# genometools/vstree

Hardware: AMD Instinct MI355X
Metric: queries/sec (100 bp queries, vmatch -mum -l 20 semantics, 3 Gbp ESA index resident in HBM) (higher is better)
Workload: dtype u8; 1 GPU; 3 Gbp synthetic DNA index, 10 M x 100 bp queries per GPU, -mum -l 20; index_bp=3000000000, queries_per_gpu=10000000, query_len=100, minlen=20, prefixlength=13, index_bytes_hbm=115012207262, reads_in_hbm=two bits per symbol, 32 bytes per read (vsa_pack_reads), parallelism=index replicated, queries sharded x1

## Files before the change

vstree_amd/csrc/api.hip:

```cpp
#include "vsa_internal.hpp"
#include <atomic>
#include <thread>
#include <time.h>
#include <algorithm>

static thread_local char g_errbuf[VSA_ERRBUF_SIZE] = "";

extern "C" char *vsa_errbuf()
{
  return g_errbuf;
}

extern "C" const char *vsa_messagespace(void)
{
  return g_errbuf;
}

int vsa_set_device(int device)
{
  VSA_HIP(hipSetDevice(device));
  return 0;
}

extern "C" int vsa_device_count(void)
// ... 411 lines not shown
    const void *from;
    uint64_t bytes;
    bool allocate;
  };
  const uint64_t ncodes = src->D > 0 ? 1ull << (2 * src->D) : 0,
                 nblocks = (n >> 6) + 1, nwaves = (nblocks + 63) / 64;
  Piece pieces[] = {
      {(void **) &ix->tis_alloc, src->tis_alloc,
       VSA_TIS_FRONTPAD + n + VSA_TIS_BACKPAD, false},
      {&ix->suf, src->suf, (n + 1) * src->isize, false},
      {(void **) &ix->lcp, src->lcp, n + 1 + 32, false},
      {&ix->llv, src->llv, 2 * src->nllv * src->isize, false},
      {&ix->bck, src->bck, 2 * src->numofcodes * src->isize, false},
      {(void **) &ix->bwt, src->bwt, n + 1 + 32, false},
      {(void **) &ix->esa8, src->esa8, (n + 1) * 8 + 64, true},
      {(void **) &ix->bck2, src->bck2, 2 * ncodes * 4 + 16, true},
      {(void **) &ix->slot16, src->slot16,
       (uint64_t) src->slotwords * ncodes * 8 + 32, true},
      {(void **) &ix->tis2, src->tis2, nblocks * 16 + 64, true},
      {(void **) &ix->spec64, src->spec64, nwaves * 8 + 64, true}};
  for (const Piece &p : pieces)
  {
    if (p.from == nullptr || p.bytes == 0)
    {
      continue;
    }
    if (p.allocate)
    {
      if (vsa_hip_malloc(p.dst, p.bytes) != hipSuccess)
      {
        VSA_ERROR("vsa_index_clone: out of device memory");
        return fail(-100);
      }
      ix->device_bytes += p.bytes;
    }
    const hipError_t e =
        hipMemcpyPeerAsync(*p.dst, device, p.from, src->device, p.bytes,
                           ix->stream);
    if (e != hipSuccess)
    {
      VSA_ERROR("vsa_index_clone: copy from device %d to device %d: %s",
                src->device, device, hipGetErrorString(e));
      return fail(-100);
    }
  }
  if (hipStreamSynchronize(ix->stream) != hipSuccess)
  {
    VSA_ERROR("vsa_index_clone: copy failed");
    return fail(-100);
  }
  ix->device_bytes = src->device_bytes;
  ix->D = src->D;
  ix->tune = src->tune;
  ix->qspeedup = src->qspeedup;
  ix->slotwords = src->slotwords;
  ix->firstspecial = src->firstspecial;
  ix->querysepposition = src->querysepposition;
  ix->hasindexedqueries = src->hasindexedqueries;
  ix->lcpquirk = src->lcpquirk;
  *clone = ix;
  return 0;
}

extern "C" void vsa_index_close(vsa_index *ix)
{
  if (ix == nullptr)
  {
    return;
  }
  (void) hipSetDevice(ix->device);
  (void) hipFree(ix->tis_alloc);
  (void) hipFree(ix->suf);
  (void) hipFree(ix->lcp);
  (void) hipFree(ix->llv);
  (void) hipFree(ix->bck);
  (void) hipFree(ix->bwt);
  (void) hipFree(ix->esa8);
  (void) hipFree(ix->bck2);
  (void) hipFree(ix->slot16);
  (void) hipFree(ix->tis2);
  (void) hipFree(ix->spec64);
  (void) hipFree(ix->isa32);
  (void) hipFree(ix->repbits);
  if (ix->stream != nullptr)
  {
    vsa_dev_forget_stream(ix->stream);
    (void) hipStreamDestroy(ix->stream);
  }
  delete ix;
}

extern "C" int vsa_index_from_tables(const vsa_tables *t, int device,
                                     vsa_index **index)
{
  if (t == nullptr || index == nullptr)
  {
    VSA_ERROR("vsa_index_from_tables: NULL argument");
    return -1;
  }
  *index = nullptr;
  if (t->integersize != 32 && t->integersize != 64)
  {
    VSA_ERROR("integersize=%u: only 32 and 64 bit indexes are supported",
              t->integersize);
    return -2;
  }
// ... 1009 lines not shown
```

vstree_amd/csrc/esa_search.hip:

```cpp
#include "search_host.hpp"
#include <rocprim/rocprim.hpp>
#include <type_traits>

#include "search_complete.inc"
#include "search_query.inc"
#include "mum_workplan.inc"
#include "mem_workplan.inc"
#include "mum_filter.inc"
#include "candidate_sort.inc"
#include <atomic>


namespace
{


enum class Form
{
  Ref,
  Deep,
  Staged,
  Rows,
  Windows
};
// ... 425 lines not shown
  rf->recsize = rf->valbits != 0 ? 4 : (rf->packed ? 8 : sizeof(vsa_match));
  return 0;
}

int compact_into(const RecordForm &form, DevBuf &raw, DevBuf &rawkeys,
                 uint64_t cap, DevBuf &cursors, DevBuf &doff, DevBuf &out,
                 DevBuf &keys, uint64_t at, hipStream_t stream)
{
  auto launch = [&](auto rec) {
    using REC = decltype(rec);
    k_compact_shards<REC><<<VSA_CURSOR_SHARDS, VSA_BLOCK, 0, stream>>>(
        raw.as<REC>(), rawkeys.as<uint64_t>(), cap,
        cursors.as<unsigned long long>(), doff.as<uint64_t>(),
        out.as<REC>() + at, keys.as<uint64_t>() + at);
  };
  if (form.valbits != 0)
  {
    launch(uint32_t());
  } else if (form.packed)
  {
    launch(uint64_t());
  } else
  {
    launch(vsa_match());
  }
  VSA_HIP(hipGetLastError());
  return 0;
}

struct QueryRun
{
  const vsa_index *index;
  const vsa_queries *queries;
  hipStream_t stream;
  DevQueries qs;
  bool domum, domumcand, ordered;
  uint32_t searchlength;
  RecordForm rec;
  Timer tall, tsearch, tfirst;
  DevBuf base;
  const uint64_t *dbase = nullptr;
  uint32_t perquery = 0;
  uint64_t nitems = 0;
  bool reduce = false, memplan = false;
  Form form = Form::Ref;
  DevBuf wcount, wtemp, wplan, wlist, wfirste, wfmlen, wfmdb, wboffset;
  const uint64_t *nlistword = nullptr;
  DevBuf pcursor, pdoff, psummary, prawout, prawkeys;
  uint64_t pcap = 0;
  bool fromplan = false, planemit = false;
  uint64_t plansearches = 0;
  DevBuf cursor, doff, summary, blocksum, rtemp, rawout, rawkeys, out, keys;
  uint64_t shardcap = 0, needed = 0, nplan = 0, nfirst = 0, plannedwork = 0;
  double searchms = 0;

  QueryRun(const vsa_index *ix, const vsa_queries *q, bool mum, bool cand,
           bool ord, uint32_t least)
      : index(ix), queries(q), stream(ix->stream), qs(devqueries(q)),
        domum(mum), domumcand(cand), ordered(ord), searchlength(least),
        tall(stream), tsearch(stream), tfirst(stream)
  {
  }
};

template <typename IDX>
int workitems(QueryRun &st)
{
  const uint64_t nqr = st.queries->nq, least = st.searchlength;
  if (st.qs.uniformlen != 0)
  {
    st.perquery = (st.qs.uniformlen >= least) ? st.qs.uniformlen - least + 1
                                              : 0;
    st.nitems = (uint64_t) st.perquery * nqr;
    return 0;
  }
  DevBuf btemp;
  auto items = rocprim::make_transform_iterator(
      rocprim::counting_iterator<uint64_t>(0),
      [len = st.qs.length, nqr, least] __device__(uint64_t q) -> uint64_t {
        if (q >= nqr)
        {
          return 0;
        }
        const uint64_t l = len[q];
        return l >= least ? l - least + 1 : 0;
      });
  if (st.base.alloc((nqr + 1) * 8))
  {
    return -100;
  }
  VSA_HIP(rocprim_run(btemp, [&](void *p, size_t &tb) {
    return rocprim::exclusive_scan(p, tb, items, st.base.as<uint64_t>(),
                                   (uint64_t) 0, (size_t) (nqr + 1),
                                   rocprim::plus<uint64_t>(), st.stream);
  }));
  st.dbase = st.base.as<uint64_t>();
  const Fetch f = {st.dbase + nqr, 8};
  return fetchwords(st.stream, &f, 1, &st.nitems) ? -100 : 0;
}

int decide(QueryRun &st)
{
  const vsa_index *index = st.index;
  const vsa_queries *queries = st.queries;
  const uint64_t maxoffsets =
      (queries->maxlength >= st.searchlength)
// ... 171 lines not shown
  if (first_pass(st, ix, st.form, bcount.as<uint64_t>()))
  {
    return -100;
  }
  VSA_HIP(rocprim_run(st.wtemp, [&](void *p, size_t &tb) {
    return rocprim::exclusive_scan(p, tb, bcount.as<uint64_t>(),
                                   st.wboffset.as<uint64_t>(), (uint64_t) 0,
                                   (size_t) (nb + 1), rocprim::plus<uint64_t>(),
                                   st.stream);
  }));
  k_wanted_fill<<<vsa_grid(nb), VSA_BLOCK, 0, st.stream>>>(
      st.wcount.as<uint32_t>(), nq, 0u, st.wboffset.as<uint64_t>(),
      st.wlist.as<uint32_t>());
  VSA_HIP(hipGetLastError());
  st.nlistword = st.wboffset.as<uint64_t>() + nb;
  PlanEmit em = PlanEmit();
  if (st.form != Form::Ref && plan_emit(st, VSA_PLAN_ROUNDS - 1, &em))
  {
    return -100;
  }
  withform(st.form, [&](auto deep, auto, auto rows, auto) {
    k_mum_plan<IDX, deep, deep, rows><<<gridfor(nq), VSA_BLOCK, 0, st.stream>>>(
        ix, st.qs, st.wlist.as<uint32_t>(), st.nlistword, st.searchlength,
        st.wfirste.as<uint32_t>(), st.wcount.as<uint32_t>(),
        st.wplan.as<PlanRanges>(), em);
  });
  if (st.planemit)
  {
    VSA_HIP(plan_summary(st));
  }
  VSA_HIP(hipGetLastError());
  const char *pf = getenv("VSA_DEBUG_PLANFILE");
  if (pf != nullptr && dump_planfile(st, pf))
  {
    return -100;
  }
  st.fromplan = true;
  return 0;
}

template <typename IDX>
void launch_search(QueryRun &st, const DevIndex<IDX> &ix,
                   uint64_t nplanblocks)
{
  withform(st.form, [&](auto deep, auto, auto rows, auto) {
    auto planned = [&](auto mum) {
      k_query_search_planned<IDX, 256, deep, rows, mum>
          <<<vsa_grid(nplanblocks), 256, 0, st.stream>>>(
              ix, st.qs, st.dbase, st.perquery, st.wplan.as<PlanRanges>(),
              st.wcount.as<uint32_t>(), st.searchlength,
              st.rawout.as<vsa_match>(), st.rawkeys.as<uint64_t>(),
              st.shardcap, VSA_CURSOR_SHARDS - 1,
              st.cursor.as<unsigned long long>(), st.rec.packbits,
              st.rec.valbits, st.blocksum.as<unsigned long long>());
    };
    auto unplanned = [&](auto mum) {
      k_query_search<IDX, mum, deep, 256>
          <<<vsa_grid((st.nitems + 255) / 256), 256, 0, st.stream>>>(
              ix, st.qs, st.dbase, st.perquery, st.nitems, st.searchlength,
              st.rawout.as<vsa_match>(), st.rawkeys.as<uint64_t>(),
              st.shardcap, VSA_CURSOR_SHARDS - 1,
              st.cursor.as<unsigned long long>(), st.rec.packbits,
              st.rec.valbits);
    };
    if (st.fromplan && st.domum)
    {
      planned(std::true_type());
    } else if (st.fromplan)
    {
      if constexpr (deep && !rows)
      {
        planned(std::false_type());
      }
    } else if (st.nitems > 0 && st.domum)
    {
      unplanned(std::true_type());
    } else if (st.nitems > 0)
    {
      unplanned(std::false_type());
    }
  });
}

template <typename IDX>
int search(QueryRun &st, const DevIndex<IDX> &ix)
{
  const uint32_t nshards = VSA_CURSOR_SHARDS;
  const uint64_t nplanblocks = (st.queries->nq + 255) / 256;
  size_t rbytes = 0;
  if (st.fromplan)
  {
    if (st.blocksum.alloc((vsa_grid_blocks(nplanblocks) + 1) * 8))
    {
      return -100;
    }
    VSA_HIP(rocprim::reduce(nullptr, rbytes,
                            st.blocksum.as<unsigned long long>(),
                            (unsigned long long *) nullptr, 0ull,
                            (size_t) nplanblocks,
                            rocprim::plus<unsigned long long>(), st.stream));
    if (st.rtemp.alloc(rbytes))
    {
      return -100;
    }
  }
  if (st.cursor.alloc((size_t) nshards * VSA_CURSOR_STRIDE * 8) ||
      st.doff.alloc(nshards * 8) || st.summary.alloc(5 * 8))
  {
    return -100;
  }
  st.shardcap =
      std::max<uint64_t>((st.queries->nq * 2 / nshards) * 5 / 4 + 64, 256);
  uint64_t maxshard = 0;
  for (int attempt = 0; attempt < 2; attempt++)
  {
    if (st.rawout.alloc(nshards * st.shardcap * st.rec.recsize) ||
        st.rawkeys.alloc(nshards * st.shardcap * 8))
    {
      return -100;
    }
    VSA_HIP(hipMemsetAsync(st.cursor.p, 0,
                           (size_t) nshards * VSA_CURSOR_STRIDE * 8,
                           st.stream));
    st.tsearch.start();
    launch_search(st, ix, nplanblocks);
    st.tsearch.stop();
    VSA_HIP(hipGetLastError());
    if (st.fromplan)
    {
      VSA_HIP(rocprim::reduce(st.rtemp.p, rbytes,
                              st.blocksum.as<unsigned long long>(),
                              st.summary.as<unsigned long long>() + 4, 0ull,
                              (size_t) nplanblocks,
                              rocprim::plus<unsigned long long>(), st.stream));
    }
    const uint64_t *sm = st.summary.as<uint64_t>();
    VSA_HIP(shard_summary(st.cursor.as<unsigned long long>(), nshards,
                          st.doff.as<uint64_t>(), st.summary.as<uint64_t>(),
                          st.stream));
    const Fetch f[7] = {{sm, 8}, {sm + 1, 8}, {sm + 2, 8}, {sm + 3, 8},
                        {sm + 4, 8}, {st.planemit ? st.psummary.p : sm, 8},
                        {st.nlistword != nullptr ? st.nlistword : sm, 8}};
    uint64_t got[7];
    if (fetchwords(st.stream, f, 7, got))
    {
      return -100;
    }
    if (st.nlistword != nullptr)
    {
      st.nfirst = got[6] >> 32;
      st.plansearches = 2 * (got[6] & 0xFFFFFFFFull);
    }
    st.nplan = st.planemit ? got[5] : 0;
    st.needed = got[0];
    maxshard = got[1];
    st.plannedwork = st.fromplan ? got[4] : 0;
    st.searchms += st.tsearch.ms();
    if (maxshard <= st.shardcap)
    {
      return 0;
    }
    st.shardcap = maxshard;
  }
  VSA_ERROR("match buffer overflow: %llu > %llu",
            (unsigned long long) maxshard, (unsigned long long) st.shardcap);
  return -5;
}

int compact(QueryRun &st)
{
  const uint64_t total = st.needed + st.nplan + st.nfirst;
  if (total == 0)
  {
    return 0;
  }
  if (st.out.alloc(total * st.rec.recsize) || st.keys.alloc(total * 8) ||
      (st.nplan > 0 &&
       compact_into(st.rec, st.prawout, st.prawkeys, st.pcap, st.pcursor,
                    st.pdoff, st.out, st.keys, st.needed, st.stream)) ||
      (st.needed > 0 &&
       compact_into(st.rec, st.rawout, st.rawkeys, st.shardcap, st.cursor,
                    st.doff, st.out, st.keys, 0, st.stream)))
  {
    return -100;
  }
  if (st.nfirst > 0)
  {
    k_append_first<<<gridfor(st.queries->nq), VSA_BLOCK, 0, st.stream>>>(
        st.wfmlen.as<uint32_t>(), st.wfmdb.as<uint64_t>(),
        st.wboffset.as<uint64_t>(), st.queries->nq, st.perquery, st.dbase,
        st.qs.seqoffset, st.needed + st.nplan, st.out.as<vsa_match>(),
        st.keys.as<uint64_t>(), st.rec.packbits, st.rec.valbits);
    VSA_HIP(hipGetLastError());
  }
  st.needed = total;
  return 0;
}

#define VSA_CS_MINPAIRS (1u << 14)

std::atomic<uint64_t> g_cs_runs{0}, g_cs_overflows{0}, g_cs_longruns{0},
    g_cs_shift{0}, g_cs_buckets{0};

bool feedsbuckets(const QueryRun &st)
{
  const uint64_t total = st.needed + st.nplan + st.nfirst;
  const uint32_t tune = st.index->tune;
  if (!(st.domum && !st.domumcand && st.rec.packed && (tune & 4u) == 0 &&
        total > 0 && (total >= VSA_CS_MINPAIRS || (tune & 8u) != 0) &&
// ... 146 lines not shown
                  bitsfor(st.nitems), st.stream))
    {
      return -100;
    }
    res->count = needed;
    res->matches = (vsa_match *) sm.release();
  }
  return 0;
}

template <typename IDX>
int run_query(const vsa_index *index, const vsa_queries *queries, bool domum,
              bool domumcand, uint32_t searchlength, vsa_result *res,
              bool ordered = true, uint32_t forcebits = 0)
{
  vsa_dev_set_stream(index->stream);
  QueryRun st(index, queries, domum, domumcand, ordered, searchlength);
  const DevIndex<IDX> ix = index->view<IDX>();
  if (workitems<IDX>(st))
  {
    return -100;
  }
  res->stats.searches = st.nitems;
  if (st.nitems == 0)
  {
    return 0;
  }
  st.tall.start();
  if (const int rc = recordform(index, queries, domum, domumcand, ordered,
                                forcebits, &st.rec))
  {
    return rc;
  }
  if (decide(st) || (st.memplan && mem_plan(st, ix)) ||
      (st.reduce && mum_plan(st, ix)))
  {
    return -100;
  }
  if (const int rc = search(st, ix))
  {
    return rc;
  }
  uint64_t mumsum = ~0ull;
  if (finish(st, res, &mumsum))
  {
    return -100;
  }
  st.tall.stop();
  VSA_HIP(hipStreamSynchronize(st.stream));
  res->stats.count = res->count;
  res->stats.search_kernel_ms = st.searchms;
  res->stats.anchor_ms = 0;
  res->stats.first_kernel_ms = st.tfirst.ms();
  res->stats.kernel_searches = st.fromplan ? st.plannedwork : st.nitems;
  if (st.fromplan)
  {
    res->stats.searches = st.plannedwork + queries->nq + st.plansearches;
  }
  res->stats.total_device_ms = st.tall.ms();
  if (mumsum != ~0ull)
  {
    res->stats.sumlength = mumsum;
    return 0;
  }
  if (st.rec.keeppairs)
  {
    res->stats.sumlength = 0;
    return 0;
  }
  return sumlengths(res->matches, res->count, st.stream,
                    &res->stats.sumlength);
}

template <typename Limits, typename Run>
int query_entry(const char *name, const vsa_index *index,
                const vsa_queries *queries, const uint64_t *searchlength,
                vsa_result **result, Limits limits, Run run)
{
  if (index == nullptr || queries == nullptr || result == nullptr)
  {
    VSA_ERROR("%s: NULL argument", name);
    return -1;
  }
  *result = nullptr;
  if (queries->device != index->device)
  {
    VSA_ERROR("queries live on device %d, index on device %d",
              queries->device, index->device);
    return -1;
  }
  if (index->bck == nullptr)
  {
    VSA_ERROR("table bck is not loaded");
    return -3;
  }
  if (searchlength != nullptr && *searchlength < index->pl)
  {
    VSA_ERROR("searchlength=%lu must be >= %lu=prefixlen",
              (unsigned long) *searchlength, (unsigned long) index->pl);
    return -2;
  }
  if (const int rc = limits())
  {
    return rc;
  }
  if (vsa_set_device(index->device) != 0)
  {
// ... 331 lines not shown
```

vstree_amd/csrc/index_derive.hip:

```cpp
#include "search_host.hpp"
#include <rocprim/rocprim.hpp>


template <typename IDX>
__global__ void __launch_bounds__(VSA_BLOCK)
k_make_esa8(const uint8_t *__restrict__ tis, const IDX *__restrict__ suf,
            const uint8_t *__restrict__ lcp, uint64_t count, uint32_t D,
            uint64_t *__restrict__ esa8)
{
  const uint64_t j = vsa_bid() * VSA_BLOCK + threadIdx.x;
  if (j >= count)
  {
    return;
  }
  const uint64_t s = suf[j];
  const uint8_t *t = tis + s + D;
  uint64_t key = 0, flag = 0;
#pragma unroll
  for (uint32_t k = 0; k < VSA_KEYSYMS; k++)
  {
    const uint8_t a = t[k];
    if (VSA_ISSPECIAL(a))
    {
      flag = VSA_KEYFLAG;
// ... 33 lines not shown
      const uint64_t packed = vsa_pack16(v.lo, v.hi);
      out[k >> 1] |= packed << (32 * (1 - (k & 1)));
    }
    out[0] = __builtin_bswap64(out[0]);
    out[1] = __builtin_bswap64(out[1]);
    reinterpret_cast<uint64_t *>(tis2)[2 * b] = out[0];
    reinterpret_cast<uint64_t *>(tis2)[2 * b + 1] = out[1];
    special = firstbad != ~0ull || 64 * b + 64 > n;
    if (firstbad != ~0ull)
    {
      atomicMin(firstspecial, (unsigned long long) firstbad);
    }
  }
  const uint64_t mask = __ballot(special);
  if ((threadIdx.x & 63) == 0 && b < nblocks)
  {
    reinterpret_cast<uint64_t *>(spec64)[b >> 6] = mask;
  }
}

template <int W, typename IDX>
__global__ void __launch_bounds__(VSA_BLOCK)
k_make_slots(const IDX *__restrict__ bck2, const uint64_t *__restrict__ esa8,
             uint64_t ncodes, uint64_t *__restrict__ slot,
             unsigned int *__restrict__ toobig)
{
  for (uint64_t c = vsa_bid() * VSA_BLOCK + threadIdx.x;
       c < ncodes; c += vsa_nblocks() * VSA_BLOCK)
  {
    const IDX left = bck2[2 * c], mid = bck2[2 * c + 1];
    if constexpr (sizeof(IDX) == 4)
    {
      slot[W * c] = (uint64_t) left | ((uint64_t) mid << 32);
    } else
    {
      const uint64_t cnt = mid > left ? mid - left : 0;
      if (cnt >> (64 - VSA_WIDE_LEFTBITS) != 0)
      {
        *toobig = 1;
      }
      slot[W * c] = left | (cnt << VSA_WIDE_LEFTBITS);
    }
#pragma unroll
    for (int k = 0; k + 1 < W; k++)
    {
      slot[W * c + 1 + k] = (mid > left + k) ? esa8[left + k] : 0;
    }
  }
}

int vsa_index_make_esa8(vsa_index *ix)
{
  const char *off = getenv("VSA_NO_ESA8");
  if (ix->esa8 != nullptr)
  {
    (void) hipFree(ix->esa8);
    ix->esa8 = nullptr;
  }
  if (ix->bck2 != nullptr)
  {
    (void) hipFree(ix->bck2);
    ix->bck2 = nullptr;
  }
  if (ix->slot16 != nullptr)
  {
    (void) hipFree(ix->slot16);
    ix->slot16 = nullptr;
  }
  if (ix->tis2 != nullptr)
  {
    (void) hipFree(ix->tis2);
    (void) hipFree(ix->spec64);
    ix->tis2 = ix->spec64 = nullptr;
  }
  const bool wide = ix->isize != 4;
  if (ix->numofchars != 4 || ix->bck == nullptr ||
      (wide && ((ix->n + 1) >> VSA_WIDE_LEFTBITS) != 0) ||
      (off != nullptr && strcmp(off, "1") == 0))
  {
    return 0;
  }
  uint32_t D = 1;
  while (D < 16 && (1ull << (2 * D)) < ix->n)
  {
    D++;
  }
  if (D < ix->pl)
  {
    D = ix->pl;
  }
  const char *fd = getenv("VSA_DEEP_PREFIX");
  if (fd != nullptr && atoi(fd) >= (int) ix->pl && atoi(fd) <= 16)
  {
    D = (uint32_t) atoi(fd);
  } else
  {
    size_t freeb = 0, totalb = 0;
    const uint32_t wanted = D;
    (void) hipStreamSynchronize(ix->stream);
    vsa_dev_trim();
    while (D > ix->pl && D > 12 &&
           hipMemGetInfo(&freeb, &totalb) == hipSuccess)
    {
      const uint64_t codes = 1ull << (2 * D),
                     need = 16 * codes + 2 * codes * ix->isize +
                            8 * (ix->n + 1) + ix->n / 4 + totalb / 10;
      if (need <= freeb)
      {
        break;
      }
      D--;
    }
    const char *tr = getenv("VSA_TRACE");
    if (tr != nullptr && strcmp(tr, "0") != 0)
    {
      fprintf(stderr, "vstree_amd: derived tables: deep prefix %u (wanted %u; "
              "%.1f GB free of %.1f on the device)\n", D, wanted,
              (double) freeb / 1e9, (double) totalb / 1e9);
    }
  }
  if (D > 16)
  {
    return 0;
  }
  static_assert(VSA_TIS_BACKPAD >= 16 + VSA_KEYSYMS + 8, "text pad too small");
  ix->D = D;
  const char *tune = getenv("VSA_TUNE");
  ix->tune = tune != nullptr ? (uint32_t) atoi(tune) : 0;
  const uint64_t count = ix->n + 1, ncodes = 1ull << (2 * D);
  VSA_HIP(hipStreamSynchronize(ix->stream));
  vsa_dev_trim();
  if (vsa_hip_malloc((void **) &ix->slot16, 2 * ncodes * 8 + 32) != hipSuccess)
  {
    (void) hipGetLastError();
    ix->slot16 = nullptr;
    ix->D = 0;
    return 0;
  }
  VSA_HIP(vsa_hip_malloc((void **) &ix->bck2, 2 * ncodes * ix->isize + 16));
  VSA_HIP(vsa_hip_malloc((void **) &ix->esa8, count * 8 + 64));
  ix->device_bytes += count * 8 + 2 * ncodes * ix->isize;
  if (wide ? vsa_build_bucket_table(ix->tis_alloc + VSA_TIS_FRONTPAD, ix->n,
                                    (const uint64_t *) ix->suf, D, 4,
                                    (uint64_t *) ix->bck2, ix->stream)
           : vsa_build_bucket_table(ix->tis_alloc + VSA_TIS_FRONTPAD, ix->n,
                                    (const uint32_t *) ix->suf, D, 4,
                                    ix->bck2, ix->stream))
  {
    return -100;
  }
  if (wide)
  {
    k_make_esa8<uint64_t><<<gridfor(count), VSA_BLOCK, 0, ix->stream>>>(
        ix->tis_alloc + VSA_TIS_FRONTPAD, (const uint64_t *) ix->suf, ix->lcp,
        count, D, ix->esa8);
  } else
  {
    k_make_esa8<uint32_t><<<gridfor(count), VSA_BLOCK, 0, ix->stream>>>(
        ix->tis_alloc + VSA_TIS_FRONTPAD, (const uint32_t *) ix->suf, ix->lcp,
        count, D, ix->esa8);
  }
  VSA_HIP(hipGetLastError());
  VSA_HIP(hipStreamSynchronize(ix->stream));
  {
    static_assert(VSA_TIS_BACKPAD >= 64, "text pad too small for k_pack_text");
    const uint64_t nblocks = (ix->n >> 6) + 1,
                   nwaves = (nblocks + 63) / 64;
    unsigned long long *dfirst = nullptr, hfirst = ix->n;
    VSA_HIP(vsa_hip_malloc((void **) &ix->tis2, nblocks * 16 + 64));
    VSA_HIP(vsa_hip_malloc((void **) &ix->spec64, nwaves * 8 + 64));
    VSA_HIP(vsa_hip_malloc((void **) &dfirst, 8));
    VSA_HIP(hipMemsetAsync(ix->tis2 + nblocks * 16, 0, 64, ix->stream));
    VSA_HIP(hipMemsetAsync(ix->spec64 + nwaves * 8, 0xFF, 64, ix->stream));
    VSA_HIP(hipMemcpyAsync(dfirst, &hfirst, 8, hipMemcpyHostToDevice,
                           ix->stream));
    k_pack_text<<<vsa_grid(nwaves * 64 / VSA_BLOCK + 1), VSA_BLOCK, 0,
                  ix->stream>>>(ix->tis_alloc + VSA_TIS_FRONTPAD, ix->n,
                                nblocks, ix->tis2, ix->spec64, dfirst);
    VSA_HIP(hipGetLastError());
    VSA_HIP(hipMemcpyAsync(&hfirst, dfirst, 8, hipMemcpyDeviceToHost,
                           ix->stream));
// ... 52 lines not shown
```

vstree_amd/csrc/mum_workplan.inc:

```



#define VSA_PLAN_RANGES 4
#define VSA_PLAN_ROUNDS 6
#define VSA_PLAN_UNKNOWN 0xFFFFFFFFu

#ifndef VSA_PLAN_WAVES
#define VSA_PLAN_WAVES 1
#endif
#ifndef VSA_FIRST_WAVES
#define VSA_FIRST_WAVES 1
#endif
struct PlanRanges
{
  uint32_t r[VSA_PLAN_RANGES];
};

__device__ __forceinline__ void plan_add(PlanRanges &pr, uint32_t &nr,
                                         uint32_t first, uint32_t last)
{
  if (first > last)
  {
    return;
  }
// ... 238 lines not shown
                             witness, hit);
      }
      if (st == VSA_LOC_SLOW)
      {
        if constexpr (ROWS)
        {
          have2 = vsa_locate_reference(ix, src + jp, qlen - jp, maxlcp2,
                                       witness);
        } else
        {
          have2 = vsa_locate_reference(ix, qstart + jp, qlen - jp, maxlcp2,
                                       witness);
        }
      } else
      {
        have2 = st == VSA_LOC_FOUND;
      }
    } else
    {
      if (doprobe)
      {
        have2 = vsa_locate_reference(ix, qstart + jp, qlen - jp, maxlcp2,
                                     witness);
      }
    }
    if (busy && have)
    {
      const bool dead = doprobe && have2 && jp + maxlcp2 == E;
      const uint32_t first = dead ? jp + 1 : j + 1;
      const uint32_t last = (E < need - 1) ? E : need - 1;
      plan_add(pr, nr, first, last);
      j = E + 1;
      busy = j < need;
    }
  }
  if (t < nlist)
  {
    if (busy)
    {
      plan_add(pr, nr, j, need - 1);
    }
    uint32_t total = 0;
#pragma unroll
    for (int i = 0; i < VSA_PLAN_RANGES; i++)
    {
      total += pr.r[i] >> 16;
    }
    plan[q] = pr;
    count[q] = total;
  }
}


#ifndef VSA_P1_WAVES
#define VSA_P1_WAVES 8
#endif
template <typename IDX, int BLK, bool DEEP = true, bool ROWS = false,
          bool MUM = true>
__global__ void __launch_bounds__(BLK, VSA_P1_WAVES)
k_query_search_planned(const DevIndex<IDX> ix, const DevQueries qs,
                       const uint64_t *__restrict__ base, uint32_t perquery,
                       const PlanRanges *__restrict__ plan,
                       const uint32_t *__restrict__ plancount,
                       uint32_t searchlength, vsa_match *__restrict__ out,
                       uint64_t *__restrict__ outkey, uint64_t shardcap,
                       uint32_t shardmask,
                       unsigned long long *__restrict__ cursors,
                       uint32_t packbits, uint32_t valbits,
                       unsigned long long *__restrict__ blocksum)
{
  __shared__ uint32_t rel[BLK + 1];
  __shared__ PlanRanges pr[BLK];
  const uint64_t q0 = vsa_bid() * BLK;
  const uint32_t tid = threadIdx.x;
  {
    const bool in = q0 + tid < qs.nq;
    const uint32_t mine = in ? plancount[q0 + tid] : 0;
    if (in)
    {
      pr[tid] = plan[q0 + tid];
    }
    rel[tid + 1] = mine;
    if (tid == 0)
    {
      rel[0] = 0;
    }
    __syncthreads();
    for (uint32_t d = 1; d < BLK; d <<= 1)
    {
      const uint32_t v = (tid + 1 > d) ? rel[tid + 1 - d] : 0;
      __syncthreads();
      rel[tid + 1] += v;
      __syncthreads();
    }
  }
  const uint32_t total = rel[BLK];
  if (tid == 0)
  {
    blocksum[vsa_bid()] = total;
  }
  const uint32_t shard = vsa_bid() & shardmask;
  for (uint32_t i0 = 0; i0 < total; i0 += BLK)
  {
    const uint32_t i = i0 + tid;
    const bool active = i < total;
    uint32_t c = 0, maxlcp = 0, off = 0, remaining = 0;
    uint64_t witness = 0, q = 0, t = 0;
    uint8_t leftchar = (uint8_t) VSA_SEPARATOR;
    const uint8_t *qptr = qs.symbols;
    bool have = false, fast = false;
    if (active)
    {
      uint32_t lo = 0, hi = BLK;
      while (hi - lo > 1)
      {
        const uint32_t mid = (lo + hi) >> 1;
        if (rel[mid] <= i)
        {
          lo = mid;
        } else
        {
          hi = mid;
        }
      }
      uint32_t r = i - rel[lo];
#pragma unroll
      for (int k = 0; k < VSA_PLAN_RANGES; k++)
      {
        const uint32_t first = pr[lo].r[k] & 0xFFFFu, len = pr[lo].r[k] >> 16;
        if (r < len)
        {
          off = first + r;
          r = 0xFFFFFFFFu;
        } else if (r != 0xFFFFFFFFu)
        {
          r -= len;
        }
      }
      q = q0 + lo;
      t = ((base != nullptr) ? base[q] : q * perquery) + off;
      if constexpr (!MUM)
      {
      } else if constexpr (ROWS)
      {
        remaining = qs.uniformlen - off;
      } else
      {
        if (qs.dense)
        {
          qptr = qs.symbols + q * qs.uniformlen + off;
          remaining = qs.uniformlen - off;
        } else
        {
          qptr = qs.symbols + qs.start[q] + off;
          remaining = (uint32_t) qs.length[q] - off;
        }
        if (off > 0)
        {
          leftchar = qptr[-1];
        }
      }
    }
    if constexpr (!MUM)
    {
      vsa_query_item<IDX, false, DEEP>(ix, qs, active, q, off, t,
                                       searchlength, out, outkey, shardcap,
                                       shard, cursors, 0, 0);
      continue;
    }
    DeepHit hit;
    int st = VSA_LOC_SLOW;
    RowQuery rq;
    QSrc src;
    if constexpr (DEEP && ROWS)
    {
      bool flagged = false;
      rq.row = qs.rows;
      rq.valid = 0;
      src.row = qs.rows;
      src.bytes = nullptr;
      src.pos = src.m = 0;
      if (active)
      {
        flagged = vsa_row_of(qs, q, qs.uniformlen, rq, src);
        if (off > 0)
        {
          leftchar = flagged ? src.bytes[off - 1]
                             : (uint8_t) (vsa_pq_window(rq, off - 1) >> 62);
        }
        src.pos = (int32_t) off;
      }
      const uint32_t qleft = off > 0 ? (uint32_t) leftchar : 0x100u;
      st = vsa_locate_deep<1, true>(ix, active && !flagged, src, remaining,
                                    maxlcp, witness, hit, searchlength, qleft,
                                    &rq, off);
      if (active && flagged)
      {
        st = VSA_LOC_SLOW;
      }
    } else if constexpr (DEEP)
    {
      st = vsa_locate_deep(ix, active, qptr, remaining, maxlcp, witness, hit,
                           searchlength,
                           off > 0 ? (uint32_t) leftchar : 0x100u);
    }
    if (st == VSA_LOC_SLOW)
    {
      if constexpr (DEEP && ROWS)
      {
        have = active &&
               vsa_locate_reference(ix, src, remaining, maxlcp, witness);
      } else
      {
        have = active &&
               vsa_locate_reference(ix, qptr, remaining, maxlcp, witness);
      }
    } else
    {
      have = st == VSA_LOC_FOUND;
      fast = have && maxlcp < 255;
    }
    if (have && maxlcp >= searchlength &&
        !(st != VSA_LOC_SLOW && hit.notleftmax))
    {
      if (fast)
      {
        const uint32_t lcpw = (uint32_t) (hit.ew >> 32) & 0xFFu;
        const bool unique = (witness == 0 || lcpw < maxlcp) &&
                            (witness + 1 > ix.n - 1 || hit.lcpnext < maxlcp);
        c = (unique && (VSA_ISSPECIAL(leftchar) || leftchar != hit.leftsym))
                ? 1u
                : 0u;
      } else
      {
        c = (vsa_mum_candidate<IDX, DEEP>(ix, maxlcp, witness) &&
             vsa_leftmaximal(ix, vsa_sufstart<IDX, DEEP>(ix, witness),
                             leftchar))
                ? 1u
                : 0u;
      }
    }
    const uint64_t inshard = vsa_wave_reserve01(
        cursors + (uint64_t) shard * VSA_CURSOR_STRIDE, c != 0);
    if (c != 0 && inshard < shardcap)
    {
      const uint64_t dbstart = fast ? vsa_entrystart(ix, hit.ew, witness)
                                    : vsa_sufstart<IDX, DEEP>(ix, witness);
      vsa_write_candidate(qs, out, outkey, (uint64_t) shard * shardcap + inshard,
                          q, off, t, dbstart, maxlcp, packbits, valbits);
    }
  }
}

template <typename IDX, bool DEEP, bool PQ = false, bool ROWS = false,
          bool WINDOWS = false>
__global__ void __launch_bounds__(VSA_BLOCK, VSA_FIRST_WAVES)
k_mum_first(const DevIndex<IDX> ix, const DevQueries qs, uint32_t perquery,
            uint32_t searchlength, uint32_t *__restrict__ count,
            uint32_t *__restrict__ firste, uint32_t *__restrict__ fmlen,
            uint64_t *__restrict__ fmdb,
            uint64_t *__restrict__ blockcount = nullptr)
{
  extern __shared__ uint32_t stagedqueries[];
  __shared__ uint32_t wantwaves[VSA_BLOCK / 64], candwaves[VSA_BLOCK / 64];
  const uint64_t q = vsa_bid() * VSA_BLOCK + threadIdx.x;
  uint32_t qlen = qs.uniformlen, perq = perquery;
  const uint8_t *qptr = qs.symbols;
  uint32_t maxlcp = 0;
  uint64_t witness = 0;
  bool have = false, fast = false;
  DeepHit hit;

  if (!ROWS && q < qs.nq)
  {
    if (qs.dense)
    {
      qptr = qs.symbols + q * qs.uniformlen;
    } else
    {
      qptr = qs.symbols + qs.start[q];
      qlen = (uint32_t) qs.length[q];
      perq = (qlen >= searchlength) ? qlen - searchlength + 1 : 0;
    }
  }
  const bool active = q < qs.nq && perq > 0;
  if constexpr (DEEP && ROWS && WINDOWS)
  {
    RowQuery rq;
    QSrc src;
    bool flagged = false;
    rq.row = qs.rows;
    rq.valid = 0;
    src.row = qs.rows;
    src.bytes = nullptr;
    src.pos = src.m = 0;
    if (q < qs.nq)
    {
      flagged = vsa_row_of(qs, q, qlen, rq, src);
    }
    int st = vsa_locate_deep<3, true>(ix, active && !flagged, src, qlen,
                                      maxlcp, witness, hit, 0xFFFFFFFFu,
                                      0x100u, &rq, 0);
// ... 216 lines not shown
```

vstree_amd/csrc/vsa_internal.hpp:

```cpp
#pragma once

#include <hip/hip_runtime.h>
#include <cstdint>
#include <cstdio>
#include <cstdlib>
#include <cstring>
#include <vector>
#include "vstree_amd.h"

extern "C" char *vsa_errbuf();
#define VSA_ERRBUF_SIZE 1024
#define VSA_ERROR(...)                                                        \
  do                                                                          \
  {                                                                           \
    snprintf(vsa_errbuf(), VSA_ERRBUF_SIZE, __VA_ARGS__);                     \
  } while (0)

#define VSA_HIP(call)                                                         \
  do                                                                          \
  {                                                                           \
    hipError_t e_ = (call);                                                   \
    if (e_ != hipSuccess)                                                     \
    {                                                                         \
      VSA_ERROR("%s:%d: %s failed: %s", __FILE__, __LINE__, #call,            \
                hipGetErrorString(e_));                                       \
      return -100;                                                            \
    }                                                                         \
  } while (0)

#define VSA_TIS_FRONTPAD 64
#define VSA_TIS_BACKPAD 64
#define VSA_QUERY_BACKPAD 64

template <typename IDX>
struct DevIndex
{
  const uint8_t *tis;
  const IDX *suf;
  const uint8_t *lcp;
  const IDX *llv;
  const IDX *bck;
  const uint8_t *bwt;
  const uint64_t *esa8;
  const uint32_t *bck2;
  const uint64_t *slot16;
  uint32_t slotwords;
  const uint8_t *tis2;
  const uint8_t *spec64;
  uint64_t firstspecial;
  uint64_t n, nllv, numofcodes;
  uint32_t pl, numofchars, D;
  uint32_t tune;
  uint32_t qspeedup;
};

#define VSA_KEYSYMS 10u
#define VSA_KEYSHIFT 40u
#define VSA_KEYMASK 0xFFFFFu
#define VSA_LEFTSHIFT 60u
#define VSA_KEYFLAG (1ull << 62)
#define VSA_LEFTSPECIAL (1ull << 63)

struct vsa_index
{
  int device;
  hipStream_t stream;
  uint32_t isize;
  uint64_t n, nllv, numofcodes;
  uint32_t pl, numofchars;
  uint8_t *tis_alloc;
  void *suf, *llv, *bck;
  uint8_t *lcp, *bwt;
  uint64_t *esa8;
  uint32_t *bck2;
  uint64_t *slot16;
  uint32_t slotwords;
  uint8_t *tis2, *spec64;
  uint64_t firstspecial;
  uint32_t D, tune;
  uint32_t qspeedup;
  uint64_t querysepposition;
  int hasindexedqueries;
  uint64_t device_bytes;
  mutable int lcpquirk;
  mutable uint32_t *isa32;
  mutable uint32_t *repbits = nullptr;
  mutable uint32_t repleast = 0;
  mutable uint32_t cs_skip = 0, cs_penalty = 0;

  template <typename IDX>
  DevIndex<IDX> view() const
  {
    DevIndex<IDX> v;
    v.tis = tis_alloc + VSA_TIS_FRONTPAD;
    v.suf = (const IDX *) suf;
    v.lcp = lcp;
    v.llv = (const IDX *) llv;
    v.bck = (const IDX *) bck;
    v.bwt = bwt;
    v.esa8 = esa8;
    v.bck2 = bck2;
    v.slot16 = slot16;
    v.slotwords = slotwords;
    v.tis2 = tis2;
    v.spec64 = spec64;
    v.firstspecial = firstspecial;
    v.D = D;
    v.tune = tune;
    v.qspeedup = qspeedup;
    v.n = n;
    v.nllv = nllv;
    v.numofcodes = numofcodes;
    v.pl = pl;
    v.numofchars = numofchars;
    return v;
  }
};

struct vsa_queries
{
  int device;
  uint64_t nq, nsymbols;
  uint64_t *rows = nullptr;
  uint32_t roww = 0;
  uint8_t *side = nullptr;
  uint64_t nside = 0;
  bool ownsrows = true;
  mutable bool bytesvalid = false;
  uint64_t bytescapacity = 0;
  mutable uint8_t *symbols;
  uint64_t *start;
  uint64_t *length;
// ... 107 lines not shown
```

Before: 3.460 billion queries/s.

## Walk MUM query offsets right-to-left in chunks, skipping offsets covered by prior matches

The planned MUM search kernel now gives each thread a chunk of up to 32 consecutive query offsets and walks them from right to left. After each locate it uses the match length to jump past offsets that cannot yield a new maximal match of the minimum length, in the style of sparse MUM scanning. Each block also handles four reads per thread, launch bounds change for the MUM variant, and the block reduction now tracks locates and offsets separately. This trades per-offset parallelism for fewer index searches, at the cost of serial dependence within a chunk, more wave divergence and higher register pressure.

```diff
diff --git a/vstree_amd/csrc/api.hip b/vstree_amd/csrc/api.hip
--- a/vstree_amd/csrc/api.hip
+++ b/vstree_amd/csrc/api.hip
@@ -487,6 +487,7 @@
   ix->device_bytes = src->device_bytes;
   ix->D = src->D;
   ix->tune = src->tune;
+  ix->walkshift = src->walkshift;
   ix->qspeedup = src->qspeedup;
   ix->slotwords = src->slotwords;
   ix->firstspecial = src->firstspecial;
diff --git a/vstree_amd/csrc/esa_search.hip b/vstree_amd/csrc/esa_search.hip
--- a/vstree_amd/csrc/esa_search.hip
+++ b/vstree_amd/csrc/esa_search.hip
@@ -501,6 +501,7 @@
   uint64_t plansearches = 0;
   DevBuf cursor, doff, summary, blocksum, rtemp, rawout, rawkeys, out, keys;
   uint64_t shardcap = 0, needed = 0, nplan = 0, nfirst = 0, plannedwork = 0;
+  uint64_t plannedlocates = 0;
   double searchms = 0;
 
   QueryRun(const vsa_index *ix, const vsa_queries *q, bool mum, bool cand,
@@ -778,7 +779,8 @@
               st.rawout.as<vsa_match>(), st.rawkeys.as<uint64_t>(),
               st.shardcap, VSA_CURSOR_SHARDS - 1,
               st.cursor.as<unsigned long long>(), st.rec.packbits,
-              st.rec.valbits, st.blocksum.as<unsigned long long>());
+              st.rec.valbits, st.blocksum.as<PlannedWork>(),
+              st.index->walkshift);
     };
     auto unplanned = [&](auto mum) {
       k_query_search<IDX, mum, deep, 256>
@@ -812,26 +814,27 @@
 int search(QueryRun &st, const DevIndex<IDX> &ix)
 {
   const uint32_t nshards = VSA_CURSOR_SHARDS;
-  const uint64_t nplanblocks = (st.queries->nq + 255) / 256;
+  const uint64_t perblock = 256 * (st.domum ? VSA_WALK_READS : 1);
+  const uint64_t nplanblocks = (st.queries->nq + perblock - 1) / perblock;
   size_t rbytes = 0;
   if (st.fromplan)
   {
-    if (st.blocksum.alloc((vsa_grid_blocks(nplanblocks) + 1) * 8))
+    if (st.blocksum.alloc((vsa_grid_blocks(nplanblocks) + 1) *
+                          sizeof(PlannedWork)))
     {
       return -100;
     }
-    VSA_HIP(rocprim::reduce(nullptr, rbytes,
-                            st.blocksum.as<unsigned long long>(),
-                            (unsigned long long *) nullptr, 0ull,
-                            (size_t) nplanblocks,
-                            rocprim::plus<unsigned long long>(), st.stream));
+    VSA_HIP(rocprim::reduce(nullptr, rbytes, st.blocksum.as<PlannedWork>(),
+                            (PlannedWork *) nullptr, PlannedWork{0, 0},
+                            (size_t) nplanblocks, PlannedWorkPlus(),
+                            st.stream));
     if (st.rtemp.alloc(rbytes))
     {
       return -100;
     }
   }
   if (st.cursor.alloc((size_t) nshards * VSA_CURSOR_STRIDE * 8) ||
-      st.doff.alloc(nshards * 8) || st.summary.alloc(5 * 8))
+      st.doff.alloc(nshards * 8) || st.summary.alloc(6 * 8))
   {
     return -100;
   }
@@ -854,21 +857,22 @@
     VSA_HIP(hipGetLastError());
     if (st.fromplan)
     {
-      VSA_HIP(rocprim::reduce(st.rtemp.p, rbytes,
-                              st.blocksum.as<unsigned long long>(),
-                              st.summary.as<unsigned long long>() + 4, 0ull,
-                              (size_t) nplanblocks,
-                              rocprim::plus<unsigned long long>(), st.stream));
+      VSA_HIP(rocprim::reduce(
+          st.rtemp.p, rbytes, st.blocksum.as<PlannedWork>(),
+          reinterpret_cast<PlannedWork *>(st.summary.as<uint64_t>() + 4),
+          PlannedWork{0, 0}, (size_t) nplanblocks, PlannedWorkPlus(),
+          st.stream));
     }
     const uint64_t *sm = st.summary.as<uint64_t>();
     VSA_HIP(shard_summary(st.cursor.as<unsigned long long>(), nshards,
                           st.doff.as<uint64_t>(), st.summary.as<uint64_t>(),
                           st.stream));
-    const Fetch f[7] = {{sm, 8}, {sm + 1, 8}, {sm + 2, 8}, {sm + 3, 8},
+    const Fetch f[8] = {{sm, 8}, {sm + 1, 8}, {sm + 2, 8}, {sm + 3, 8},
                         {sm + 4, 8}, {st.planemit ? st.psummary.p : sm, 8},
-                        {st.nlistword != nullptr ? st.nlistword : sm, 8}};
-    uint64_t got[7];
-    if (fetchwords(st.stream, f, 7, got))
+                        {st.nlistword != nullptr ? st.nlistword : sm, 8},
+                        {sm + 5, 8}};
+    uint64_t got[8];
+    if (fetchwords(st.stream, f, 8, got))
     {
       return -100;
     }
@@ -880,7 +884,8 @@
     st.nplan = st.planemit ? got[5] : 0;
     st.needed = got[0];
     maxshard = got[1];
-    st.plannedwork = st.fromplan ? got[4] : 0;
+    st.plannedlocates = st.fromplan ? got[4] : 0;
+    st.plannedwork = st.fromplan ? got[7] : 0;
     st.searchms += st.tsearch.ms();
     if (maxshard <= st.shardcap)
     {
@@ -1133,7 +1138,7 @@
   res->stats.search_kernel_ms = st.searchms;
   res->stats.anchor_ms = 0;
   res->stats.first_kernel_ms = st.tfirst.ms();
-  res->stats.kernel_searches = st.fromplan ? st.plannedwork : st.nitems;
+  res->stats.kernel_searches = st.fromplan ? st.plannedlocates : st.nitems;
   if (st.fromplan)
   {
     res->stats.searches = st.plannedwork + queries->nq + st.plansearches;
diff --git a/vstree_amd/csrc/index_derive.hip b/vstree_amd/csrc/index_derive.hip
--- a/vstree_amd/csrc/index_derive.hip
+++ b/vstree_amd/csrc/index_derive.hip
@@ -109,6 +109,25 @@
 int vsa_index_make_esa8(vsa_index *ix)
 {
   const char *off = getenv("VSA_NO_ESA8");
+  {
+    const char *tn = getenv("VSA_TUNE"), *wc = getenv("VSA_WALK_CHUNK");
+    const int asked = wc != nullptr ? atoi(wc) : 0;
+    ix->tune = tn != nullptr ? (uint32_t) atoi(tn) : 0;
+    uint32_t chunk = VSA_WALK_CHUNK;
+    if (asked >= 1 && asked <= 0x8000)
+    {
+      chunk = (uint32_t) asked;
+    }
+    if ((ix->tune & 16u) != 0)
+    {
+      chunk = 1;
+    }
+    ix->walkshift = 0;
+    while ((2u << ix->walkshift) <= chunk)
+    {
+      ix->walkshift++;
+    }
+  }
   if (ix->esa8 != nullptr)
   {
     (void) hipFree(ix->esa8);
@@ -182,8 +201,6 @@
   }
   static_assert(VSA_TIS_BACKPAD >= 16 + VSA_KEYSYMS + 8, "text pad too small");
   ix->D = D;
-  const char *tune = getenv("VSA_TUNE");
-  ix->tune = tune != nullptr ? (uint32_t) atoi(tune) : 0;
   const uint64_t count = ix->n + 1, ncodes = 1ull << (2 * D);
   VSA_HIP(hipStreamSynchronize(ix->stream));
   vsa_dev_trim();
diff --git a/vstree_amd/csrc/mum_walk.inc b/vstree_amd/csrc/mum_walk.inc
--- /dev/null
+++ b/vstree_amd/csrc/mum_walk.inc
@@ -0,0 +1,111 @@
+template <typename IDX, bool DEEP, bool PQ, typename QP>
+__device__ __forceinline__ uint32_t
+vsa_walk_chunk(const DevIndex<IDX> &ix, const DevQueries &qs, bool active,
+               QP read, const RowQuery *rq, uint32_t qlen, uint32_t first,
+               uint32_t off, uint64_t q, const uint64_t *__restrict__ base,
+               uint32_t perquery, uint32_t searchlength,
+               vsa_match *__restrict__ out, uint64_t *__restrict__ outkey,
+               uint64_t shardcap, uint32_t shard,
+               unsigned long long *__restrict__ cursors, uint32_t packbits,
+               uint32_t valbits)
+{
+  uint32_t locates = 0;
+  while (__any(active))
+  {
+    uint32_t c = 0, maxlcp = 0;
+    uint64_t witness = 0;
+    uint8_t leftchar = (uint8_t) VSA_SEPARATOR;
+    const uint32_t remaining = qlen - off;
+    const QP qptr = read + off;
+    bool have = false, fast = false;
+    DeepHit hit;
+    int st = VSA_LOC_SLOW;
+    locates += active ? 1u : 0u;
+    if (active && off > 0)
+    {
+      if constexpr (PQ)
+      {
+        leftchar = (uint8_t) (vsa_pq_window(*rq, off - 1) >> 62);
+      } else
+      {
+        leftchar = vsa_qsym(read, off - 1);
+      }
+    }
+    if constexpr (DEEP)
+    {
+      const uint32_t qleft = off > 0 ? (uint32_t) leftchar : 0x100u;
+      if constexpr (PQ)
+      {
+        st = vsa_locate_deep<1, true>(ix, active, qptr, remaining, maxlcp,
+                                      witness, hit, searchlength, qleft, rq,
+                                      off);
+      } else
+      {
+        st = vsa_locate_deep(ix, active, qptr, remaining, maxlcp, witness,
+                             hit, searchlength, qleft);
+      }
+    }
+    if (st == VSA_LOC_SLOW)
+    {
+      have = active &&
+             vsa_locate_reference(ix, qptr, remaining, maxlcp, witness);
+    } else
+    {
+      have = st == VSA_LOC_FOUND;
+      fast = have && maxlcp < 255;
+    }
+    const bool cutshort = st != VSA_LOC_SLOW && hit.notleftmax;
+    if (have && maxlcp >= searchlength && !cutshort)
+    {
+      if (fast)
+      {
+        const uint32_t lcpw = (uint32_t) (hit.ew >> 32) & 0xFFu;
+        const bool unique = (witness == 0 || lcpw < maxlcp) &&
+                            (witness + 1 > ix.n - 1 || hit.lcpnext < maxlcp);
+        c = (unique && (VSA_ISSPECIAL(leftchar) || leftchar != hit.leftsym))
+                ? 1u
+                : 0u;
+      } else
+      {
+        c = (vsa_mum_candidate<IDX, DEEP>(ix, maxlcp, witness) &&
+             vsa_leftmaximal(ix, vsa_sufstart<IDX, DEEP>(ix, witness),
+                             leftchar))
+                ? 1u
+                : 0u;
+      }
+    }
+    const uint64_t inshard = vsa_wave_reserve01(
+        cursors + (uint64_t) shard * VSA_CURSOR_STRIDE, c != 0);
+    if (c != 0 && inshard < shardcap)
+    {
+      const uint64_t dbstart = fast ? vsa_entrystart(ix, hit.ew, witness)
+                                    : vsa_sufstart<IDX, DEEP>(ix, witness);
+      const uint64_t t0 = (base != nullptr) ? base[q] : q * perquery;
+      vsa_write_candidate(qs, out, outkey,
+                          (uint64_t) shard * shardcap + inshard, q, off,
+                          t0 + off, dbstart, maxlcp, packbits, valbits);
+    }
+    if (active)
+    {
+      uint32_t bound;
+      if (st == VSA_LOC_SLOW)
+      {
+        bound = have ? maxlcp : ix.pl - 1;
+      } else
+      {
+        bound = have ? maxlcp : ix.D - 1;
+      }
+      const uint32_t reach = off + bound;
+      uint32_t next = off - 1;
+      bool left = off > first;
+      if (!cutshort && reach + 1 < off + searchlength)
+      {
+        left = left && reach >= searchlength;
+        next = reach - searchlength;
+      }
+      active = left && next >= first;
+      off = next;
+    }
+  }
+  return locates;
+}
diff --git a/vstree_amd/csrc/mum_workplan.inc b/vstree_amd/csrc/mum_workplan.inc
--- a/vstree_amd/csrc/mum_workplan.inc
+++ b/vstree_amd/csrc/mum_workplan.inc
@@ -314,12 +314,33 @@
 }
 
 
+#include "mum_walk.inc"
+
+struct PlannedWork
+{
+  unsigned long long locates, offsets;
+};
+struct PlannedWorkPlus
+{
+  __host__ __device__ PlannedWork operator()(const PlannedWork &a,
+                                             const PlannedWork &b) const
+  {
+    return PlannedWork{a.locates + b.locates, a.offsets + b.offsets};
+  }
+};
+
 #ifndef VSA_P1_WAVES
 #define VSA_P1_WAVES 8
 #endif
+#ifndef VSA_WALK_WAVES
+#define VSA_WALK_WAVES 6
+#endif
+#ifndef VSA_WALK_READS
+#define VSA_WALK_READS 4
+#endif
 template <typename IDX, int BLK, bool DEEP = true, bool ROWS = false,
           bool MUM = true>
-__global__ void __launch_bounds__(BLK, VSA_P1_WAVES)
+__global__ void __launch_bounds__(BLK, MUM ? VSA_WALK_WAVES : VSA_P1_WAVES)
 k_query_search_planned(const DevIndex<IDX> ix, const DevQueries qs,
                        const uint64_t *__restrict__ base, uint32_t perquery,
                        const PlanRanges *__restrict__ plan,
@@ -329,12 +350,18 @@
                        uint32_t shardmask,
                        unsigned long long *__restrict__ cursors,
                        uint32_t packbits, uint32_t valbits,
-                       unsigned long long *__restrict__ blocksum)
-{
-  __shared__ uint32_t rel[BLK + 1];
-  __shared__ PlanRanges pr[BLK];
-  const uint64_t q0 = vsa_bid() * BLK;
+                       PlannedWork *__restrict__ blocksum,
+                       uint32_t chunkshift = 0)
+{
+  constexpr int RPT = MUM ? VSA_WALK_READS : 1, RPB = BLK * RPT;
+  __shared__ uint32_t rel[RPB + 1];
+  __shared__ PlanRanges pr[RPB];
+  __shared__ uint64_t lanesum[MUM ? BLK + 1 : 1];
+  __shared__ uint32_t wavelocates[MUM ? BLK / 64 : 1];
+  const uint64_t q0 = vsa_bid() * RPB;
   const uint32_t tid = threadIdx.x;
+  const uint32_t cshift = MUM ? chunkshift : 0, chunk = 1u << cshift;
+  if constexpr (!MUM)
   {
     const bool in = q0 + tid < qs.nq;
     const uint32_t mine = in ? plancount[q0 + tid] : 0;
@@ -355,25 +382,76 @@
       rel[tid + 1] += v;
       __syncthreads();
     }
-  }
-  const uint32_t total = rel[BLK];
+  } else
+  {
+    uint32_t mine[RPT], sum = 0, offsets = 0;
+#pragma unroll
+    for (int k = 0; k < RPT; k++)
+    {
+      const uint64_t q = q0 + tid * RPT + k;
+      uint32_t c = q < qs.nq ? plancount[q] : 0;
+      offsets += c;
+      if (q < qs.nq)
+      {
+        const PlanRanges p = plan[q];
+        pr[tid * RPT + k] = p;
+        if (c > 0)
+        {
+          c = 0;
+#pragma unroll
+          for (int g = 0; g < VSA_PLAN_RANGES; g++)
+          {
+            c += ((p.r[g] >> 16) + chunk - 1) >> cshift;
+          }
+        }
+      }
+      sum += c;
+      mine[k] = sum;
+    }
+    lanesum[tid + 1] = sum | ((uint64_t) offsets << 32);
+    if (tid == 0)
+    {
+      lanesum[0] = 0;
+      rel[0] = 0;
+    }
+    __syncthreads();
+    for (uint32_t d = 1; d < BLK; d <<= 1)
+    {
+      const uint64_t v = (tid + 1 > d) ? lanesum[tid + 1 - d] : 0;
+      __syncthreads();
+      lanesum[tid + 1] += v;
+      __syncthreads();
+    }
+#pragma unroll
+    for (int k = 0; k < RPT; k++)
+    {
+      rel[tid * RPT + k + 1] = (uint32_t) lanesum[tid] + mine[k];
+    }
+    __syncthreads();
+  }
+  const uint32_t total = rel[RPB];
   if (tid == 0)
   {
-    blocksum[vsa_bid()] = total;
+    if constexpr (MUM)
+    {
+      blocksum[vsa_bid()].offsets = lanesum[BLK] >> 32;
+    } else
+    {
+      blocksum[vsa_bid()] = PlannedWork{total, total};
+    }
   }
   const uint32_t shard = vsa_bid() & shardmask;
+  uint32_t locates = 0;
   for (uint32_t i0 = 0; i0 < total; i0 += BLK)
   {
     const uint32_t i = i0 + tid;
-    const bool active = i < total;
-    uint32_t c = 0, maxlcp = 0, off = 0, remaining = 0;
-    uint64_t witness = 0, q = 0, t = 0;
-    uint8_t leftchar = (uint8_t) VSA_SEPARATOR;
-    const uint8_t *qptr = qs.symbols;
-    bool have = false, fast = false;
+    bool active = i < total;
+    uint32_t off = 0, first = 0, qlen = qs.uniformlen;
+    uint64_t q = 0, t0 = 0;
+    const uint8_t *qstart = qs.symbols;
     if (active)
     {
-      uint32_t lo = 0, hi = BLK;
+      uint32_t lo = 0, hi = RPB;
       while (hi - lo > 1)
       {
         const uint32_t mid = (lo + hi) >> 1;
@@ -389,53 +467,48 @@
 #pragma unroll
       for (int k = 0; k < VSA_PLAN_RANGES; k++)
       {
-        const uint32_t first = pr[lo].r[k] & 0xFFFFu, len = pr[lo].r[k] >> 16;
-        if (r < len)
-        {
-          off = first + r;
+        const uint32_t rf = pr[lo].r[k] & 0xFFFFu, len = pr[lo].r[k] >> 16,
+                       nchunks = (len + chunk - 1) >> cshift;
+        if (r < nchunks)
+        {
+          const uint32_t at = r << cshift,
+                         n = len - at < chunk ? len - at : chunk;
+          first = rf + at;
+          off = first + n - 1;
           r = 0xFFFFFFFFu;
         } else if (r != 0xFFFFFFFFu)
         {
-          r -= len;
+          r -= nchunks;
         }
       }
       q = q0 + lo;
-      t = ((base != nullptr) ? base[q] : q * perquery) + off;
       if constexpr (!MUM)
       {
-      } else if constexpr (ROWS)
-      {
-        remaining = qs.uniformlen - off;
-      } else
+        t0 = (base != nullptr) ? base[q] : q * perquery;
+      }
+      if constexpr (MUM && !ROWS)
       {
         if (qs.dense)
         {
-          qptr = qs.symbols + q * qs.uniformlen + off;
-          remaining = qs.uniformlen - off;
+          qstart = qs.symbols + q * qs.uniformlen;
         } else
         {
-          qptr = qs.symbols + qs.start[q] + off;
-          remaining = (uint32_t) qs.length[q] - off;
-        }
-        if (off > 0)
-        {
-          leftchar = qptr[-1];
+          qstart = qs.symbols + qs.start[q];
+          qlen = (uint32_t) qs.length[q];
         }
       }
     }
     if constexpr (!MUM)
     {
-      vsa_query_item<IDX, false, DEEP>(ix, qs, active, q, off, t,
+      vsa_query_item<IDX, false, DEEP>(ix, qs, active, q, off, t0 + off,
                                        searchlength, out, outkey, shardcap,
                                        shard, cursors, 0, 0);
       continue;
     }
-    DeepHit hit;
-    int st = VSA_LOC_SLOW;
-    RowQuery rq;
-    QSrc src;
     if constexpr (DEEP && ROWS)
     {
+      RowQuery rq;
+      QSrc src;
       bool flagged = false;
       rq.row = qs.rows;
       rq.valid = 0;
@@ -445,71 +518,47 @@
       if (active)
       {
         flagged = vsa_row_of(qs, q, qs.uniformlen, rq, src);
-        if (off > 0)
-        {
-          leftchar = flagged ? src.bytes[off - 1]
-                             : (uint8_t) (vsa_pq_window(rq, off - 1) >> 62);
-        }
-        src.pos = (int32_t) off;
-      }
-      const uint32_t qleft = off > 0 ? (uint32_t) leftchar : 0x100u;
-      st = vsa_locate_deep<1, true>(ix, active && !flagged, src, remaining,
-                                    maxlcp, witness, hit, searchlength, qleft,
-                                    &rq, off);
-      if (active && flagged)
-      {
-        st = VSA_LOC_SLOW;
-      }
-    } else if constexpr (DEEP)
-    {
-      st = vsa_locate_deep(ix, active, qptr, remaining, maxlcp, witness, hit,
-                           searchlength,
-                           off > 0 ? (uint32_t) leftchar : 0x100u);
-    }
-    if (st == VSA_LOC_SLOW)
-    {
-      if constexpr (DEEP && ROWS)
-      {
-        have = active &&
-               vsa_locate_reference(ix, src, remaining, maxlcp, witness);
-      } else
-      {
-        have = active &&
-               vsa_locate_reference(ix, qptr, remaining, maxlcp, witness);
-      }
-    } else
-    {
-      have = st == VSA_LOC_FOUND;
-      fast = have && maxlcp < 255;
-    }
-    if (have && maxlcp >= searchlength &&
-        !(st != VSA_LOC_SLOW && hit.notleftmax))
-    {
-      if (fast)
-      {
-        const uint32_t lcpw = (uint32_t) (hit.ew >> 32) & 0xFFu;
-        const bool unique = (witness == 0 || lcpw < maxlcp) &&
-                            (witness + 1 > ix.n - 1 || hit.lcpnext < maxlcp);
-        c = (unique && (VSA_ISSPECIAL(leftchar) || leftchar != hit.leftsym))
-                ? 1u
-                : 0u;
-      } else
-      {
-        c = (vsa_mum_candidate<IDX, DEEP>(ix, maxlcp, witness) &&
-             vsa_leftmaximal(ix, vsa_sufstart<IDX, DEEP>(ix, witness),
-                             leftchar))
-                ? 1u
-                : 0u;
-      }
-    }
-    const uint64_t inshard = vsa_wave_reserve01(
-        cursors + (uint64_t) shard * VSA_CURSOR_STRIDE, c != 0);
-    if (c != 0 && inshard < shardcap)
-    {
-      const uint64_t dbstart = fast ? vsa_entrystart(ix, hit.ew, witness)
-                                    : vsa_sufstart<IDX, DEEP>(ix, witness);
-      vsa_write_candidate(qs, out, outkey, (uint64_t) shard * shardcap + inshard,
-                          q, off, t, dbstart, maxlcp, packbits, valbits);
+      }
+      locates += vsa_walk_chunk<IDX, true, true>(
+          ix, qs, active && !flagged, src, &rq, qlen, first, off, q, base,
+          perquery, searchlength, out, outkey, shardcap, shard, cursors,
+          packbits, valbits);
+      if (__any(active && flagged))
+      {
+        locates += vsa_walk_chunk<IDX, true, false>(
+            ix, qs, active && flagged, src, nullptr, qlen, first, off, q, base,
+            perquery, searchlength, out, outkey, shardcap, shard, cursors,
+            packbits, valbits);
+      }
+    } else
+    {
+      locates += vsa_walk_chunk<IDX, DEEP, false>(
+          ix, qs, active, qstart, nullptr, qlen, first, off, q, base, perquery,
+          searchlength, out, outkey, shardcap, shard, cursors, packbits,
+          valbits);
+    }
+  }
+  if constexpr (MUM)
+  {
+#pragma unroll
+    for (int d = 32; d >= 1; d >>= 1)
+    {
+      locates += __shfl_xor(locates, d, 64);
+    }
+    if ((tid & 63u) == 0)
+    {
+      wavelocates[tid >> 6] = locates;
+    }
+    __syncthreads();
+    if (tid == 0)
+    {
+      uint32_t s = 0;
+#pragma unroll
+      for (int w = 0; w < BLK / 64; w++)
+      {
+        s += wavelocates[w];
+      }
+      blocksum[vsa_bid()].locates = s;
     }
   }
 }
diff --git a/vstree_amd/csrc/vsa_internal.hpp b/vstree_amd/csrc/vsa_internal.hpp
--- a/vstree_amd/csrc/vsa_internal.hpp
+++ b/vstree_amd/csrc/vsa_internal.hpp
@@ -61,6 +61,10 @@
 #define VSA_KEYFLAG (1ull << 62)
 #define VSA_LEFTSPECIAL (1ull << 63)
 
+#ifndef VSA_WALK_CHUNK
+#define VSA_WALK_CHUNK 32
+#endif
+
 struct vsa_index
 {
   int device;
@@ -78,6 +82,7 @@
   uint8_t *tis2, *spec64;
   uint64_t firstspecial;
   uint32_t D, tune;
+  uint32_t walkshift;
   uint32_t qspeedup;
   uint64_t querysepposition;
   int hasindexedqueries;
```

After: 3.796 billion queries/s (median of 6 runs). +9.7%, better.
